# guiga-zalu/pixlzr-rust

Hardware: AMD Instinct MI355X
Metric: encode megapixels/sec (per-tile LOD detection + block-wise downsample), 8K RGBA (higher is better)
Workload: dtype u8

## Files before the change

### pixlzr-rust_amd/csrc/pxz_device.h

```cpp
#pragma once
#include <hip/hip_runtime.h>
#include <stdint.h>
#include <stdlib.h>

#include "pxz_internal.h"

namespace pxz {


static __constant__ uint32_t kSrgbToLinearBits[256] = {
#include "srgb_lut.inc"
};

struct RecipAlphaTable {
	uint32_t v[256];
	constexpr RecipAlphaTable() : v{}
	{
		for (uint32_t a = 1; a < 256; ++a) v[a] = ((255u * 512u) / a + 1u) >> 1;
	}
};
static __constant__ RecipAlphaTable kRecipAlpha = RecipAlphaTable();


__device__ __forceinline__ uint32_t fastdiv(uint32_t n, const FastDiv &d)
// ... 519 lines not shown
}

template <int C = 4>
__device__ __forceinline__ void resample_fast16_hv(const uint32_t *trows, const AxisTab &tx, const AxisTab &ty, const uint32_t *s_pl,
                                                   uint32_t *s_tmp, uint32_t lane, uint32_t nw, uint32_t nh, uint32_t *out)
{
	const uint32_t lgx = 31u - (uint32_t)__builtin_clz(nw);
	if (nw >= 4) {
		switch (tx.wquads) {
		case 1: fast32_h_pairs<1>(trows, tx, s_pl, s_tmp, lane, nw, lgx, 8u); break;
		case 2: fast32_h_pairs<2>(trows, tx, s_pl, s_tmp, lane, nw, lgx, 8u); break;
		case 3: fast32_h_pairs<3>(trows, tx, s_pl, s_tmp, lane, nw, lgx, 8u); break;
		default: fast32_h_pairs<4>(trows, tx, s_pl, s_tmp, lane, nw, lgx, 8u); break;
		}
	} else if (nw == 2) {
		fast32_h_rows<2>(trows, tx, s_pl, s_tmp, lane, nw, lgx, 16u);
	} else {
		fast32_h_rows<4>(trows, tx, s_pl, s_tmp, lane, nw, lgx, 16u);
	}
	tile_sync<1>();
	const uint32_t items = nw * nh;
	if (items >= 64u) fast32_v<1, C>(trows, tx, ty, s_tmp, lane, nw, nh, out);
	else if (items >= 32u) fast32_v<2, C>(trows, tx, ty, s_tmp, lane, nw, nh, out);
	else if (items >= 16u) fast32_v<4, C>(trows, tx, ty, s_tmp, lane, nw, nh, out);
	else fast32_v<8, C>(trows, tx, ty, s_tmp, lane, nw, nh, out);
	tile_sync<1>();
}

typedef int v4i32 __attribute__((ext_vector_type(4)));
typedef float f32x2 __attribute__((ext_vector_type(2)));

template <int BYTE>
__device__ __forceinline__ void put_byte_shr(uint32_t &dst, uint32_t value, uint32_t shift)
{
	if constexpr (BYTE == 0)
		asm("v_lshrrev_b32_sdwa %0, %1, %2 dst_sel:BYTE_0 dst_unused:UNUSED_PRESERVE src0_sel:DWORD src1_sel:DWORD" : "+v"(dst) : "v"(shift), "v"(value));
	else if constexpr (BYTE == 1)
		asm("v_lshrrev_b32_sdwa %0, %1, %2 dst_sel:BYTE_1 dst_unused:UNUSED_PRESERVE src0_sel:DWORD src1_sel:DWORD" : "+v"(dst) : "v"(shift), "v"(value));
	else if constexpr (BYTE == 2)
		asm("v_lshrrev_b32_sdwa %0, %1, %2 dst_sel:BYTE_2 dst_unused:UNUSED_PRESERVE src0_sel:DWORD src1_sel:DWORD" : "+v"(dst) : "v"(shift), "v"(value));
	else
		asm("v_lshrrev_b32_sdwa %0, %1, %2 dst_sel:BYTE_3 dst_unused:UNUSED_PRESERVE src0_sel:DWORD src1_sel:DWORD" : "+v"(dst) : "v"(shift), "v"(value));
}

__device__ __forceinline__ uint32_t clamp_fixed(int32_t hi, int32_t lo, int32_t top)
{
	const int32_t v = (int32_t)(((uint32_t)hi << 8) + (uint32_t)lo);
	int32_t r;
	asm("v_med3_i32 %0, %1, 0, %2" : "=v"(r) : "v"(v), "s"(top));
	return (uint32_t)r;
}

template <int NCH>
__device__ __forceinline__ void resample_mfma32(const uint32_t *s_tab, const AxisTab &tx, const AxisTab &ty, const uint32_t *s_pl,
                                                uint32_t lane, uint32_t nw, uint32_t nh, uint32_t *out)
{
	const uint32_t o = lane & 15u, g = lane >> 4;
	const uint32_t *mx = s_tab + tx.mf_off, *my = s_tab + ty.mf_off;
	const long kx_lo = *reinterpret_cast<const long *>(mx + 2u * lane), kx_hi = *reinterpret_cast<const long *>(mx + 128u + 2u * lane);
	const long ky_lo = *reinterpret_cast<const long *>(my + 2u * lane), ky_hi = *reinterpret_cast<const long *>(my + 128u + 2u * lane);
	const int32_t bx = (int32_t)mx[256u + o];
	const v4i32 cx = {bx, bx, bx, bx};
	const v4i32 cy = *reinterpret_cast<const v4i32 *>(my + 256u + 4u * g);
	const v4i32 zero = {0, 0, 0, 0};
	const uint32_t px_ = tx.precision, py = ty.precision;
	const int32_t top_x = (int32_t)((256u << px_) - 1u), top_y = (int32_t)((256u << py) - 1u);
	uint32_t pix[4] = {0xff000000u, 0xff000000u, 0xff000000u, 0xff000000u};
	const uint32_t *rowp = s_pl + o * kRS32 + 2u * g;
#pragma unroll
	for (uint32_t c = 0; c < (uint32_t)NCH; ++c) {
		uint32_t t[2];
#pragma unroll
		for (uint32_t mb = 0; mb < 2; ++mb) {
			const uint32_t *row = rowp + c * kPD32 + mb * (16u * kRS32);
			const uint2 d0 = lds_load2(row);
			const uint2 d1 = lds_load2(row + 8u);
			const uint32_t a0 = __builtin_amdgcn_perm(d0.y, d0.x, 0x06040200u) ^ 0x80808080u;
			const uint32_t a1 = __builtin_amdgcn_perm(d1.y, d1.x, 0x06040200u) ^ 0x80808080u;
			const long av = (long)(((unsigned long long)a1 << 32) | (unsigned long long)a0);
			const v4i32 lo = __builtin_amdgcn_mfma_i32_16x16x32_i8(av, kx_lo, cx, 0, 0, 0);
			const v4i32 hi = __builtin_amdgcn_mfma_i32_16x16x32_i8(av, kx_hi, zero, 0, 0, 0);
			uint32_t packed = 0;
			put_byte_shr<0>(packed, clamp_fixed(hi[0], lo[0], top_x), px_);
			put_byte_shr<1>(packed, clamp_fixed(hi[1], lo[1], top_x), px_);
			put_byte_shr<2>(packed, clamp_fixed(hi[2], lo[2], top_x), px_);
			put_byte_shr<3>(packed, clamp_fixed(hi[3], lo[3], top_x), px_);
			t[mb] = packed ^ 0x80808080u;
		}
		const long tv = (long)(((unsigned long long)t[1] << 32) | (unsigned long long)t[0]);
		const v4i32 lo = __builtin_amdgcn_mfma_i32_16x16x32_i8(ky_lo, tv, cy, 0, 0, 0);
		const v4i32 hi = __builtin_amdgcn_mfma_i32_16x16x32_i8(ky_hi, tv, zero, 0, 0, 0);
#pragma unroll
		for (int r = 0; r < 4; ++r) {
			const uint32_t v = clamp_fixed(hi[r], lo[r], top_y);
			if (c == 0) put_byte_shr<0>(pix[r], v, py);
			else if (c == 1) put_byte_shr<1>(pix[r], v, py);
			else if (c == 2) put_byte_shr<2>(pix[r], v, py);
			else put_byte_shr<3>(pix[r], v, py);
		}
	}
	if constexpr (NCH == 4) {
#pragma unroll
		for (int r = 0; r < 4; ++r) pix[r] = unpremultiply(pix[r]);
	} else if (!(mx[288] & my[288])) {
		const int32_t ah = (int32_t)clip8((1 << (px_ - 1)) + 255 * (int32_t)mx[272u + o], (int)px_);
#pragma unroll
		for (int r = 0; r < 4; ++r) {
			const uint32_t al = clip8((1 << (py - 1)) + ah * (int32_t)my[272u + 4u * g + (uint32_t)r], (int)py);
			pix[r] = (pix[r] & 0x00ffffffu) | (al << 24);
			if (al != 255u) pix[r] = unpremultiply(pix[r]);
		}
	}
	if (o < nw) {
#pragma unroll
		for (uint32_t r = 0; r < 4; ++r) {
			const uint32_t oy = 4u * g + r;
			if (oy < nh) out[oy * nw + o] = pix[r];
		}
	}
}

__device__ __forceinline__ void resample_mfma32_narrow(const uint32_t *s_tab, const AxisTab &tx, const AxisTab &ty, const uint32_t *s_pl,
                                                       uint32_t lane, uint32_t nw, uint32_t nh, uint32_t *out)
{
	const uint32_t o = lane & 15u, g = lane >> 4;
	const uint32_t lgw = nw >> 1;
	const uint32_t ch = o >> lgw, ox = o & (nw - 1u);
	const uint32_t *mx = s_tab + tx.mf_off, *my = s_tab + ty.mf_off;
	const uint32_t own = 2u * (16u * g + ox), none = 2u * (16u * g + 15u);
	const long ky_lo = *reinterpret_cast<const long *>(my + 2u * lane), ky_hi = *reinterpret_cast<const long *>(my + 128u + 2u * lane);
	const uint32_t px_ = tx.precision, py = ty.precision;
	const int32_t top_x = (int32_t)((256u << px_) - 1u), top_y = (int32_t)((256u << py) - 1u);
	const int32_t bx = ch == 3u ? top_x : (int32_t)mx[256u + ox];
	const v4i32 cy = *reinterpret_cast<const v4i32 *>(my + 256u + 4u * g);
	const v4i32 zero = {0, 0, 0, 0};
	v4i32 lo[2] = {{bx, bx, bx, bx}, {bx, bx, bx, bx}}, hi[2] = {zero, zero};
	const uint32_t *rowp = s_pl + o * kRS32 + 2u * g;
#pragma unroll
	for (uint32_t c = 0; c < 3; ++c) {
		const uint32_t sel = ch == c ? own : none;
		const long k_lo = *reinterpret_cast<const long *>(mx + sel), k_hi = *reinterpret_cast<const long *>(mx + 128u + sel);
#pragma unroll
		for (uint32_t mb = 0; mb < 2; ++mb) {
			const uint32_t *row = rowp + c * kPD32 + mb * (16u * kRS32);
			const uint2 d0 = lds_load2(row);
			const uint2 d1 = lds_load2(row + 8u);
			const uint32_t a0 = __builtin_amdgcn_perm(d0.y, d0.x, 0x06040200u) ^ 0x80808080u;
			const uint32_t a1 = __builtin_amdgcn_perm(d1.y, d1.x, 0x06040200u) ^ 0x80808080u;
			const long av = (long)(((unsigned long long)a1 << 32) | (unsigned long long)a0);
			lo[mb] = __builtin_amdgcn_mfma_i32_16x16x32_i8(av, k_lo, lo[mb], 0, 0, 0);
			hi[mb] = __builtin_amdgcn_mfma_i32_16x16x32_i8(av, k_hi, hi[mb], 0, 0, 0);
		}
	}
	uint32_t t[2];
#pragma unroll
	for (uint32_t mb = 0; mb < 2; ++mb) {
		uint32_t packed = 0;
		put_byte_shr<0>(packed, clamp_fixed(hi[mb][0], lo[mb][0], top_x), px_);
		put_byte_shr<1>(packed, clamp_fixed(hi[mb][1], lo[mb][1], top_x), px_);
		put_byte_shr<2>(packed, clamp_fixed(hi[mb][2], lo[mb][2], top_x), px_);
		put_byte_shr<3>(packed, clamp_fixed(hi[mb][3], lo[mb][3], top_x), px_);
		t[mb] = packed ^ 0x80808080u;
	}
	const long tv = (long)(((unsigned long long)t[1] << 32) | (unsigned long long)t[0]);
	const v4i32 vlo = __builtin_amdgcn_mfma_i32_16x16x32_i8(ky_lo, tv, cy, 0, 0, 0);
	const v4i32 vhi = __builtin_amdgcn_mfma_i32_16x16x32_i8(ky_hi, tv, zero, 0, 0, 0);
	if (o < 4u * nw && 4u * g < nh) {
		uint8_t *dst = reinterpret_cast<uint8_t *>(out) + (4u * g * nw + ox) * 4u + ch;
		dst[0] = (uint8_t)(clamp_fixed(vhi[0], vlo[0], top_y) >> py);
		if (nh > 1u) dst[nw * 4u] = (uint8_t)(clamp_fixed(vhi[1], vlo[1], top_y) >> py);
		if (nh > 2u) {
			dst[2u * nw * 4u] = (uint8_t)(clamp_fixed(vhi[2], vlo[2], top_y) >> py);
			dst[3u * nw * 4u] = (uint8_t)(clamp_fixed(vhi[3], vlo[3], top_y) >> py);
		}
	}
}

__device__ __forceinline__ uint32_t clamp_fixed_v(int32_t hi, int32_t lo, int32_t top)
{
	const int32_t v = (int32_t)(((uint32_t)hi << 8) + (uint32_t)lo);
	int32_t r;
	asm("v_med3_i32 %0, %1, 0, %2" : "=v"(r) : "v"(v), "v"(top));
	return (uint32_t)r;
}
// ... 46 lines not shown
			const v4i32 cx = {bx[mb], bx[mb], bx[mb], bx[mb]};
			const v4i32 lo = __builtin_amdgcn_mfma_i32_16x16x32_i8(av, kx_lo[mb], cx, 0, 0, 0);
			const v4i32 hi = __builtin_amdgcn_mfma_i32_16x16x32_i8(av, kx_hi[mb], zero, 0, 0, 0);
			uint32_t packed = 0;
			put_byte_shr<0>(packed, clamp_fixed_v(hi[0], lo[0], top_x[mb]), px_[mb]);
			put_byte_shr<1>(packed, clamp_fixed_v(hi[1], lo[1], top_x[mb]), px_[mb]);
			put_byte_shr<2>(packed, clamp_fixed_v(hi[2], lo[2], top_x[mb]), px_[mb]);
			put_byte_shr<3>(packed, clamp_fixed_v(hi[3], lo[3], top_x[mb]), px_[mb]);
			t[mb] = packed ^ 0x80808080u;
		}
		const uint32_t l0 = second ? 0u : t[0], l1 = second ? 0u : t[1], r0 = second ? t[0] : 0u, r1 = second ? t[1] : 0u;
		const long tl = (long)(((unsigned long long)l1 << 32) | (unsigned long long)l0);
		const long tr = (long)(((unsigned long long)r1 << 32) | (unsigned long long)r0);
		v4i32 lo = __builtin_amdgcn_mfma_i32_16x16x32_i8(ky_lo[0], tl, cy, 0, 0, 0);
		lo = __builtin_amdgcn_mfma_i32_16x16x32_i8(ky_lo[1], tr, lo, 0, 0, 0);
		v4i32 hi = __builtin_amdgcn_mfma_i32_16x16x32_i8(ky_hi[0], tl, zero, 0, 0, 0);
		hi = __builtin_amdgcn_mfma_i32_16x16x32_i8(ky_hi[1], tr, hi, 0, 0, 0);
#pragma unroll
		for (int r = 0; r < 4; ++r) {
			const uint32_t v = clamp_fixed_v(hi[r], lo[r], top_y);
			if (c == 0) put_byte_shr<0>(pix[r], v, py);
			else if (c == 1) put_byte_shr<1>(pix[r], v, py);
			else put_byte_shr<2>(pix[r], v, py);
		}
	}
	if (ok && o < nw) {
#pragma unroll
		for (uint32_t r = 0; r < 4; ++r) {
			const uint32_t oy = 4u * (g & 1u) + r;
			if (oy < nh) store_pixel<C>(dst, oy * nw + o, pix[r]);
		}
	}
}

__device__ __forceinline__ uint4 stream_load4(const uint8_t *p)
{
	typedef uint32_t u32q __attribute__((ext_vector_type(4)));
	const u32q v = __builtin_nontemporal_load(reinterpret_cast<const u32q *>(p));
	return make_uint4(v.x, v.y, v.z, v.w);
}
__device__ __forceinline__ uint2 stream_load2(const uint8_t *p)
{
	typedef uint32_t u32d __attribute__((ext_vector_type(2)));
	const u32d v = __builtin_nontemporal_load(reinterpret_cast<const u32d *>(p));
	return make_uint2(v.x, v.y);
}
__device__ __forceinline__ uint3 stream_load3(const uint8_t *p)
{
	typedef uint32_t u32t __attribute__((ext_vector_type(3)));
	const u32t v = __builtin_nontemporal_load(reinterpret_cast<const u32t *>(p));
	return make_uint3(v.x, v.y, v.z);
}

template <int C = 4, class Args>
__device__ __forceinline__ bool fast32_tile_src(const Args &a, uint32_t tile_g, const uint8_t *&src)
{
	if (tile_g >= a.n_tiles) return false;
	const uint32_t frame = fastdiv(tile_g, a.div_tpf);
	const uint32_t t = tile_g - frame * a.tiles_per_frame;
	const uint32_t ty = fastdiv(t, a.div_cols), tx = t - ty * a.cols;
	src = a.src + (size_t)frame * a.frame_stride + (size_t)(ty * 32u) * a.pitch + (size_t)(tx * 32u) * (uint32_t)C;
	return tx < a.full_cols && ty < a.full_rows;
}
template <int C = 4, class Args>
__device__ __forceinline__ void fast32_prefetch(const Args &a, uint32_t tile_g, uint32_t lane, uint4 (&pre)[4], bool &valid, bool skip_loads = false)
{
	const uint8_t *src;
	valid = fast32_tile_src<C>(a, tile_g, src);
	if (valid && !skip_loads) {
		const uint8_t *p = src + (size_t)(lane >> 3) * a.pitch + (lane & 7u) * (4u * (uint32_t)C);
#pragma unroll
		for (int k = 0; k < 4; ++k) {
			if constexpr (C == 4) {
				pre[k] = stream_load4(p + (size_t)(8 * k) * a.pitch);
			} else {
				const uint3 v = stream_load3(p + (size_t)(8 * k) * a.pitch);
				pre[k] = make_uint4(v.x, v.y, v.z, 0u);
			}
		}
	}
}

template <class Args>
__device__ __forceinline__ bool oklab_value_given(const Args &a, uint32_t tx, uint32_t ty)
{
	const bool in_x = tx < a.full_cols, in_y = ty < a.full_rows;
	if (in_x && ty < a.ok_rows) return true;
	const uint32_t bit = in_x ? 2u : (in_y ? 1u : 4u);
	return (a.ok_edges & bit) != 0u;
}

constexpr uint32_t kDeferredKey = 0xffffffffu;
__device__ __forceinline__ void finish_tile(const uint2 key, uint32_t w, uint32_t h, uint32_t mode, float factor, float *value,
                                            float *lod0, float *lod1, uint32_t tile_g)
{
	float raw0, raw1, v0, v1;
	if (mode == 1) {
		const uint64_t fac = (uint64_t)(w - 2) * (uint64_t)(h - 2) * 4096ull;
		if (fac == 0) {
			raw0 = raw1 = __uint_as_float(0xFFC00000u);
			v0 = v1 = 0.0f;
		} else {
			const double d = (double)fac;
			raw0 = (float)((double)key.x / d);
			raw1 = (float)((double)key.y / d);
			v0 = parse_value(raw0 * factor);
			v1 = parse_value(raw1 * factor);
		}
	} else {
		raw0 = raw1 = __uint_as_float(key.x);
		v0 = v1 = parse_value(raw0);
	}
	if (value) value[tile_g] = hypot_f32(v0, v1);
	if (lod0) lod0[tile_g] = raw0;
	if (lod1) lod1[tile_g] = raw1;
}

#ifdef PXZ_STAMPS
__device__ __forceinline__ unsigned long long stamp_now()
{
	unsigned long long t;
	__builtin_amdgcn_sched_barrier(0);
	asm volatile("s_memtime %0\n\ts_waitcnt lgkmcnt(0)" : "=s"(t)::"memory");
	__builtin_amdgcn_sched_barrier(0);
	return t;
}
#define PXZ_STAMP(i)                                   \
	do {                                               \
		const unsigned long long now_ = stamp_now();   \
		st_acc[i] += now_ - st_last;                   \
		st_last = now_;                                \
	} while (0)
#else
// ... 241 lines not shown
```

### pixlzr-rust_amd/csrc/pxz_shrink32.hip

```cpp
#include "pxz_device.h"

namespace pxz {


template <int MODE, bool FULL, int C = 4>
__global__ void __launch_bounds__(1024) shrink32_kernel(const Fast32Args a)
{
	extern __shared__ __attribute__((aligned(16))) uint32_t lds[];
	const uint32_t wpb = blockDim.x / 64u, sub = threadIdx.x / 64u, tid = threadIdx.x % 64u;
	for (uint32_t i = threadIdx.x; i < a.tab_dw / 4u; i += blockDim.x)
		reinterpret_cast<uint4 *>(lds)[i] = reinterpret_cast<const uint4 *>(a.trows)[i];
	uint32_t *s_ticket = lds + a.tab_dw + wpb * a.tile_dw;
	if (threadIdx.x == 0) *s_ticket = wpb;
	__syncthreads();
	const uint32_t *s_tab = lds;
	const uint32_t brk_lane = tid < (uint32_t)kMaxLevel ? a.breaks[tid] : (a.breaks_asc ? 0xffffffffu : 0u);
	auto level_of = [&](uint32_t key) -> uint32_t {
		const unsigned long long lt = __builtin_amdgcn_ballot_w64(key < brk_lane);
		const unsigned long long live = (1ull << kMaxLevel) - 1ull;
		return (uint32_t)__builtin_popcountll((a.breaks_asc ? ~lt : lt) & live);
	};
	uint32_t *s_pl = lds + a.tab_dw + sub * a.tile_dw;
	uint32_t *s_tmp = s_pl + 3 * kPD32;
	uint32_t *s_batch = s_ticket + 4u + sub * (2u * kListBatch);
	uint32_t n_listb = 0, n_lista = 0;
	auto tile_of_ticket = [&](uint32_t t) -> uint32_t {
		const unsigned long long run = (unsigned long long)(t >> a.chunk_lg) * gridDim.x + blockIdx.x;
		const unsigned long long g = (run << a.chunk_lg) + (t & ((1u << a.chunk_lg) - 1u));
		return g < (unsigned long long)a.n_tiles ? (uint32_t)g : 0xffffffffu;
	};
	auto next_ticket = [&]() -> uint32_t {
		uint32_t t = 0;
		if (tid == 0) t = atomicAdd(s_ticket, 1u);
		return tile_of_ticket(__builtin_amdgcn_readfirstlane(t));
	};
	uint4 pre[4];
	bool pre_valid = false;
	const uint32_t first = tile_of_ticket(__builtin_amdgcn_readfirstlane(sub));
	bool pre_skipped = false;
	uint32_t vb_cur = 0, vb_next = 0;
	uint32_t fl_next = 0;
	auto value_pair_of = [&](uint32_t t) -> uint2 { return t < a.n_tiles ? reinterpret_cast<const uint2 *>(a.sums)[t] : make_uint2(0u, 0u); };
	auto stored_whole = [&](uint32_t vb, uint32_t copied) -> bool {
		return a.clone_ahead && copied == 1u && level_of(__float_as_uint(parse_value(__uint_as_float(vb)))) == 0u;
	};
	uint32_t second = 0xffffffffu;
	if constexpr (MODE == 0) {
		second = next_ticket();
		const uint2 p0 = value_pair_of(first), p1 = value_pair_of(second);
		vb_cur = __builtin_amdgcn_readfirstlane(p0.x);
		vb_next = __builtin_amdgcn_readfirstlane(p1.x);
		fl_next = __builtin_amdgcn_readfirstlane(p1.y);
		pre_skipped = stored_whole(vb_cur, __builtin_amdgcn_readfirstlane(p0.y));
		fast32_prefetch<C>(a, first, tid, pre, pre_valid, pre_skipped);
	} else {
		fast32_prefetch<C>(a, first, tid, pre, pre_valid);
	}
#ifdef PXZ_STAMPS
	unsigned long long st_acc[8] = {0, 0, 0, 0, 0, 0, 0, 0};
	unsigned long long st_last = stamp_now();
	const unsigned long long st_begin = wall_clock64();
#endif
	uint32_t pend_kind = 0;
	uint32_t pend_px = 0;
	const uint32_t *pend_src = nullptr;
	uint8_t *pend_dst = nullptr;
	auto flush = [&]() {
		if (pend_kind == 1) {
			if constexpr (C == 4) {
				uint32_t *d = reinterpret_cast<uint32_t *>(pend_dst);
				if (pend_px >= 4u) {
					for (uint32_t i = tid; i < (pend_px >> 2); i += 64u)
						reinterpret_cast<uint4 *>(d)[i] = reinterpret_cast<const uint4 *>(pend_src)[i];
				} else if (tid < pend_px) {
					d[tid] = pend_src[tid];
				}
			} else {
				if (pend_px >= 4u) {
					for (uint32_t i = tid; i < (pend_px >> 2); i += 64u) {
						const uint4 v = reinterpret_cast<const uint4 *>(pend_src)[i];
						uint3 o;
						o.x = __builtin_amdgcn_perm(v.y, v.x, 0x04020100u);
						o.y = __builtin_amdgcn_perm(v.z, v.y, 0x05040201u);
						o.z = __builtin_amdgcn_perm(v.w, v.z, 0x06050402u);
						reinterpret_cast<uint3 *>(pend_dst)[i] = o;
					}
				} else if (tid < pend_px) {
					const uint32_t v = pend_src[tid];
					pend_dst[3u * tid] = (uint8_t)v;
					pend_dst[3u * tid + 1u] = (uint8_t)(v >> 8);
					pend_dst[3u * tid + 2u] = (uint8_t)(v >> 16);
				}
			}
		} else if (pend_kind == 2) {
#pragma unroll
			for (int k = 0; k < 4; ++k) {
				const uint32_t i = tid + 64u * (uint32_t)k;
				const uint32_t *p = s_pl + (i >> 3) * kRS32 + (i & 7u) * 2u;
				const uint2 r = *reinterpret_cast<const uint2 *>(p), g = *reinterpret_cast<const uint2 *>(p + kPD32);
				const uint2 b = *reinterpret_cast<const uint2 *>(p + 2 * kPD32);
				const uint32_t rg01 = __builtin_amdgcn_perm(g.x, r.x, 0x06020400u), rg23 = __builtin_amdgcn_perm(g.y, r.y, 0x06020400u);
				if constexpr (C == 4) {
					const uint32_t opq = 0x00ff00ffu;
					const uint32_t ba01 = __builtin_amdgcn_perm(opq, b.x, 0x06020400u), ba23 = __builtin_amdgcn_perm(opq, b.y, 0x06020400u);
					uint4 o;
					o.x = __builtin_amdgcn_perm(ba01, rg01, 0x05040100u);
					o.y = __builtin_amdgcn_perm(ba01, rg01, 0x07060302u);
					o.z = __builtin_amdgcn_perm(ba23, rg23, 0x05040100u);
					o.w = __builtin_amdgcn_perm(ba23, rg23, 0x07060302u);
					reinterpret_cast<uint4 *>(pend_dst)[i] = o;
				} else {
					uint3 o;
					o.x = __builtin_amdgcn_perm(b.x, rg01, 0x02040100u);
					const uint32_t gb1 = __builtin_amdgcn_perm(b.x, rg01, 0x0c0c0603u);
					o.y = __builtin_amdgcn_perm(rg23, gb1, 0x05040100u);
					o.z = __builtin_amdgcn_perm(b.y, rg23, 0x06030204u);
					reinterpret_cast<uint3 *>(pend_dst)[i] = o;
				}
			}
		}
		pend_kind = 0;
	};
	auto one_tile = [&](const uint32_t tile_g, const uint32_t tile_next) {
		auto prefetch_next = [&]() __attribute__((always_inline)) {
			if constexpr (MODE == 0) {
				pre_skipped = stored_whole(vb_next, fl_next);
				fast32_prefetch<C>(a, tile_next, tid, pre, pre_valid, pre_skipped);
			} else {
				fast32_prefetch<C>(a, tile_next, tid, pre, pre_valid);
			}
		};
		auto defer = [&]() {
			list_push(s_batch, n_listb, tile_g, a.work + kWorkList, a.work + a.work_slot, tid);
			if (tid == 0) {
				bool keep = false;
				if constexpr (MODE == 0) {
					const uint32_t t = tile_g - fastdiv(tile_g, a.div_tpf) * a.tiles_per_frame;
					const uint32_t ty = fastdiv(t, a.div_cols), tx = t - ty * a.cols;
					keep = oklab_value_given(a, tx, ty);
				}
				if (!keep) reinterpret_cast<uint2 *>(a.sums)[tile_g] = make_uint2(kDeferredKey, kDeferredKey);
			}
		};
		if (!pre_valid) {
			flush();
			defer();
			prefetch_next();
			return;
		}
		uint32_t given_bits = 0;
		if constexpr (MODE == 0) given_bits = vb_cur;
		const bool skipped = MODE == 0 && pre_skipped;
		bool transparent = false;
		if (C == 4 && !skipped) {
			uint32_t least;
			const uint32_t m0 = min(min(pre[0].x, pre[0].y), pre[0].z), m1 = min(min(pre[0].w, pre[1].x), pre[1].y);
			const uint32_t m2 = min(min(pre[1].z, pre[1].w), pre[2].x), m3 = min(min(pre[2].y, pre[2].z), pre[2].w);
			const uint32_t m4 = min(min(pre[3].x, pre[3].y), pre[3].z);
			least = min(min(min(m0, m1), m2), min(min(m3, m4), pre[3].w));
			transparent = __builtin_amdgcn_ballot_w64(least < 0xff000000u) != 0ull;
		}
		__builtin_amdgcn_sched_barrier(0);
		flush();
		__builtin_amdgcn_sched_barrier(0);
		if (!skipped) {
#pragma unroll
		for (int k = 0; k < 4; ++k) {
			const uint32_t row = (tid >> 3) + 8u * (uint32_t)k, col = tid & 7u;
			const uint4 v = pre[k];
			uint32_t *d = s_pl + row * kRS32 + col * 2u;
			if constexpr (C == 4) {
#pragma unroll
				for (uint32_t c = 0; c < 3; ++c) {
					const uint32_t sel = c | 0x0c000c00u | ((4u + c) << 16);
					uint2 pr;
					pr.x = __builtin_amdgcn_perm(v.y, v.x, sel);
					pr.y = __builtin_amdgcn_perm(v.w, v.z, sel);
					lds_store2(d + c * kPD32, pr);
				}
			} else {
				lds_store2(d, make_uint2(__builtin_amdgcn_perm(v.x, v.x, 0x0c070c00u), __builtin_amdgcn_perm(v.z, v.y, 0x0c050c02u)));
				lds_store2(d + kPD32, make_uint2(__builtin_amdgcn_perm(v.y, v.x, 0x0c040c01u), __builtin_amdgcn_perm(v.z, v.y, 0x0c060c03u)));
				lds_store2(d + 2 * kPD32, make_uint2(__builtin_amdgcn_perm(v.y, v.x, 0x0c050c02u), __builtin_amdgcn_perm(v.z, v.z, 0x0c070c00u)));
			}
		}
		}
		PXZ_STAMP(0);
		prefetch_next();
		if (skipped) {
			uint32_t lane = tid;
			asm volatile("" : "+v"(lane));
			if (lane == 0) {
				if (FULL || a.out_w) a.out_w[tile_g] = 32u;
				if (FULL || a.out_h) a.out_h[tile_g] = 32u;
			}
			return;
		}
		if (transparent && (FULL || a.out_px != nullptr)) {
			if (a.alpha_list) {
				list_push(s_batch + kListBatch, n_lista, tile_g, a.work + kWorkList + a.n_tiles, a.work + kWorkA + a.work_slot, tid);
				if constexpr (MODE == 1)
					if (tid == 0) reinterpret_cast<uint2 *>(a.sums)[tile_g] = make_uint2(kDeferredKey, kDeferredKey);
			} else {
				defer();
			}
			return;
		}
		tile_sync<1>();
		PXZ_STAMP(1);

		uint32_t m0, m1;
		uint32_t key0 = 0, key1 = 0;
		if constexpr (MODE == 1) {
			uint32_t sum_hz = 0, sum_vr = 0;
			const uint32_t q = tid & 15u, g = tid >> 4;
			auto last_rows = [](uint32_t grp) -> bool {
				asm volatile("" : "+v"(grp));
				return grp != 3u;
			};
			const uint32_t two = 0x00020002u;
			const uint32_t *pc[3];
			pc[0] = s_pl + g * (8u * kRS32) + q;
			pc[1] = pc[0] + kPD32;
			pc[2] = pc[1] + kPD32;
			uint32_t rA[3], rB[3], tP[3], dP[3];
#pragma unroll
			for (int c = 0; c < 3; ++c) {
				const uint32_t a0 = lds_dword(pc[0] + c * kPD32), a1 = lds_dword(pc[0] + c * kPD32 + 1);
				const uint32_t b0 = lds_dword(pc[0] + c * kPD32 + kRS32), b1 = lds_dword(pc[0] + c * kPD32 + kRS32 + 1);
				rA[c] = pk_mad_u16(__builtin_amdgcn_alignbit(a1, a0, 16), two, add2x16(a0, a1));
				rB[c] = pk_mad_u16(__builtin_amdgcn_alignbit(b1, b0, 16), two, add2x16(b0, b1));
				tP[c] = add2x16(a0, b0);
				dP[c] = b0;
			}
#pragma unroll
			for (int st = 0; st < 4; ++st) {
				if (st < 3 || last_rows(g)) {
#pragma unroll
					for (int c = 0; c < 3; ++c) {
						const uint32_t *pr = pc[0] + c * kPD32 + (2 + 2 * st) * (int)kRS32;
						const uint32_t n0 = lds_dword(pr), n1 = lds_dword(pr + 1), o0 = lds_dword(pr + kRS32), o1 = lds_dword(pr + kRS32 + 1);
						const uint32_t rN = pk_mad_u16(__builtin_amdgcn_alignbit(n1, n0, 16), two, add2x16(n0, n1));
						sum_hz = sad16(rN, rA[c], sum_hz);
						const uint32_t tN = add2x16(dP[c], n0);
						const uint32_t c0 = add2x16(tP[c], tN);
						sum_vr = sad16(dpp_mov<0x101>(c0), c0, sum_vr);
						const uint32_t rO = pk_mad_u16(__builtin_amdgcn_alignbit(o1, o0, 16), two, add2x16(o0, o1));
						sum_hz = sad16(rO, rB[c], sum_hz);
						const uint32_t tO = add2x16(n0, o0);
						const uint32_t e0 = add2x16(tN, tO);
						sum_vr = sad16(dpp_mov<0x101>(e0), e0, sum_vr);
						rA[c] = rN;
						rB[c] = rO;
						tP[c] = tO;
						dP[c] = o0;
					}
				}
			}
			{
				uint32_t qq = q;
				asm volatile("" : "+v"(qq));
				if (qq == 15u) sum_hz = sum_vr = 0;
			}
			sum_hz = wave_sum_sgpr(sum_hz);
			sum_vr = wave_sum_sgpr(sum_vr);
			m0 = level_of(sum_hz);
			m1 = level_of(sum_vr);
			key0 = sum_hz;
			key1 = sum_vr;
		} else {
			m0 = m1 = level_of(__float_as_uint(parse_value(__uint_as_float(given_bits))));
		}
		const uint32_t nw = reduced_size(32u, m0), nh = reduced_size(32u, m1);
		{
			uint32_t lane = tid;
			asm volatile("" : "+v"(lane));
			if (lane == 0) {
				if constexpr (MODE == 1) reinterpret_cast<uint2 *>(a.sums)[tile_g] = make_uint2(key0, key1);
				if (FULL || a.out_w) a.out_w[tile_g] = nw;
				if (FULL || a.out_h) a.out_h[tile_g] = nh;
			}
		}
		PXZ_STAMP(2);
		if (FULL || a.out_px != nullptr) {
			uint32_t filt = a.filter;
			asm volatile("" : "+s"(filt));
			pend_dst = a.out_px + (size_t)tile_g * (1024u * (uint32_t)C);
			pend_px = nw * nh;
			if (nw == 32u && nh == 32u) {
				pend_kind = 2;
			} else if (nw != 32u && nh != 32u && filt != 0) {
				const uint32_t lx = m0 < (uint32_t)kMaxLevel ? m0 : (uint32_t)kMaxLevel - 1;
				const uint32_t ly = m1 < (uint32_t)kMaxLevel ? m1 : (uint32_t)kMaxLevel - 1;
				const bool both_mf = a.tabs[lx].mf_off != 0 && a.tabs[ly].mf_off != 0;
				if (a.narrow && both_mf && nw <= 4u && nh <= 16u && (s_tab[a.tabs[lx].mf_off + 288u] & s_tab[a.tabs[ly].mf_off + 288u])) {
					resample_mfma32_narrow(s_tab, a.tabs[lx], a.tabs[ly], s_pl, tid, nw, nh, s_tmp);
					pend_src = s_tmp;
					pend_kind = 1;
				} else if (both_mf && nw >= 4u && nh >= 4u) {
					resample_mfma32<3>(s_tab, a.tabs[lx], a.tabs[ly], s_pl, tid, nw, nh, s_tmp);
					pend_src = s_tmp;
					pend_kind = 1;
				} else if (nw <= 8u) {
					resample_fast32_hv(s_tab, a.tabs[lx], a.tabs[ly], s_pl, s_tmp, tid, nw, nh, s_pl);
					pend_src = s_pl;
					pend_kind = 1;
				} else {
					defer();
				}
			} else if (filt == 0) {
				const uint32_t lgx = 31u - (uint32_t)__builtin_clz(nw);
				const uint32_t hx = m0 ? (1u << (m0 < 6u ? m0 - 1u : 4u)) : 0u, hy = m1 ? (1u << (m1 < 6u ? m1 - 1u : 4u)) : 0u;
				const uint16_t *pl16 = reinterpret_cast<const uint16_t *>(s_pl);
				for (uint32_t i = tid; i < nw * nh; i += 64u) {
					const uint32_t ox = i & (nw - 1u), oy = i >> lgx;
					const uint32_t x = m0 == 0 ? ox : (m0 < 6u ? (2u * ox + 1u) * hx : 16u);
					const uint32_t y = m1 == 0 ? oy : (m1 < 6u ? (2u * oy + 1u) * hy : 16u);
					const uint32_t idx = y * (2u * kRS32) + x;
					s_tmp[i] = (uint32_t)pl16[idx] | ((uint32_t)pl16[idx + 2u * kPD32] << 8) | ((uint32_t)pl16[idx + 4u * kPD32] << 16) | 0xff000000u;
				}
				pend_kind = 1;
				pend_src = s_tmp;
			} else if (nh != 32u) {
				const uint32_t ly = m1 < (uint32_t)kMaxLevel ? m1 : (uint32_t)kMaxLevel - 1;
				fast32_v_only(s_tab, a.tabs[ly], s_pl, tid, nh, s_tmp);
				pend_kind = 1;
				pend_src = s_tmp;
			} else {
				const uint32_t lx = m0 < (uint32_t)kMaxLevel ? m0 : (uint32_t)kMaxLevel - 1;
				fast32_h_only(s_tab, a.tabs[lx], s_pl, tid, nw, s_tmp);
				pend_kind = 1;
				pend_src = s_tmp;
			}
		}
		tile_sync<1>();
		PXZ_STAMP(3);
	};
#ifdef PXZ_STAMPS
	uint32_t st_tiles = 0;
#endif
	for (uint32_t tile_g = first, tile_next = second; tile_g < a.n_tiles;) {
#ifdef PXZ_STAMPS
		++st_tiles;
#endif
		if constexpr (MODE == 0) {
			const uint32_t tile_after = next_ticket();
			const uint2 pair_after = value_pair_of(tile_after);
			one_tile(tile_g, tile_next);
			tile_g = tile_next;
			tile_next = tile_after;
			vb_cur = vb_next;
			vb_next = __builtin_amdgcn_readfirstlane(pair_after.x);
			fl_next = __builtin_amdgcn_readfirstlane(pair_after.y);
		} else {
			tile_next = next_ticket();
			one_tile(tile_g, tile_next);
			tile_g = tile_next;
		}
	}
#ifdef PXZ_STAMPS
	unsigned long long st_loop_end;
	asm volatile("s_memrealtime %0\n\ts_waitcnt lgkmcnt(0)" : "=s"(st_loop_end)::"memory");
#endif
	flush();
	list_flush(s_batch, n_listb, a.work + kWorkList, a.work + a.work_slot, tid);
	list_flush(s_batch + kListBatch, n_lista, a.work + kWorkList + a.n_tiles, a.work + kWorkA + a.work_slot, tid);
	if (a.finish_here) {
		__threadfence_block();
		__syncthreads();
		for (uint32_t i = threadIdx.x;; i += blockDim.x) {
			const unsigned long long run = (unsigned long long)(i >> a.chunk_lg) * gridDim.x + blockIdx.x;
			const unsigned long long g = (run << a.chunk_lg) + (i & ((1u << a.chunk_lg) - 1u));
			if (g >= (unsigned long long)a.n_tiles) break;
			const uint2 key = reinterpret_cast<const uint2 *>(a.sums)[g];
			if (key.x == kDeferredKey && key.y == kDeferredKey) continue;
			finish_tile(key, 32u, 32u, (uint32_t)MODE, a.factor, a.value, a.lod0, a.lod1, (uint32_t)g);
		}
	}
#ifdef PXZ_STAMPS
	if (tid == 0) {
		unsigned long long *out = reinterpret_cast<unsigned long long *>(a.work + ((2u * a.n_tiles + kWorkList + 1u + 1u) & ~1u));
		for (int i = 0; i < 8; ++i) atomicAdd(out + i, st_acc[i]);
// ... 20 lines not shown
		const unsigned long long live = (1ull << kMaxLevel) - 1ull;
		return (uint32_t)__builtin_popcountll((a.breaks_asc ? ~lt : lt) & live);
	};
	uint32_t *s_pl = lds + a.tab_dw + sub * a.tile_dw;
	uint32_t *s_batch = s_ticket + 4u + sub * kListBatch;
	uint32_t n_listb = 0;
	const uint32_t count = a.all_tiles ? a.n_tiles : __builtin_amdgcn_readfirstlane(a.work[kWorkA + a.work_slot]);
	const uint32_t *list = a.work + kWorkList + a.n_tiles;
	uint32_t n_transparent = 0;
	auto tile_of_ticket = [&](uint32_t t) -> uint32_t {
		const unsigned long long i = (unsigned long long)blockIdx.x + (unsigned long long)t * gridDim.x;
		return i < (unsigned long long)count ? (a.all_tiles ? (uint32_t)i : list[(uint32_t)i]) : 0xffffffffu;
	};
	auto next_ticket = [&]() -> uint32_t {
		uint32_t t = 0;
		if (tid == 0) t = atomicAdd(s_ticket, 1u);
		return __builtin_amdgcn_readfirstlane(tile_of_ticket(__builtin_amdgcn_readfirstlane(t)));
	};
	uint4 pre[4];
	bool pre_valid = false;
	const uint32_t first = __builtin_amdgcn_readfirstlane(tile_of_ticket(__builtin_amdgcn_readfirstlane(sub)));
	fast32_prefetch(a, first, tid, pre, pre_valid);
	for (uint32_t tile_g = first; tile_g < a.n_tiles;) {
		const uint32_t tile_next = next_ticket();
		auto defer = [&]() {
			list_push(s_batch, n_listb, tile_g, a.work + kWorkList, a.work + a.work_slot, tid);
		};
		if (!pre_valid) {
			if (tid == 0) {
				bool keep = false;
				if constexpr (MODE == 0) {
					const uint32_t t = tile_g - fastdiv(tile_g, a.div_tpf) * a.tiles_per_frame;
					const uint32_t ty = fastdiv(t, a.div_cols), tx = t - ty * a.cols;
					keep = oklab_value_given(a, tx, ty);
				}
				if (!keep) reinterpret_cast<uint2 *>(a.sums)[tile_g] = make_uint2(kDeferredKey, kDeferredKey);
			}
			defer();
			fast32_prefetch(a, tile_next, tid, pre, pre_valid);
			tile_g = tile_next;
			continue;
		}
		uint32_t given_bits = 0;
		if constexpr (MODE == 0) given_bits = a.sums[2 * tile_g];
		if (a.all_tiles) {
			const uint32_t m0 = min(min(pre[0].x, pre[0].y), pre[0].z), m1 = min(min(pre[0].w, pre[1].x), pre[1].y);
			const uint32_t m2 = min(min(pre[1].z, pre[1].w), pre[2].x), m3 = min(min(pre[2].y, pre[2].z), pre[2].w);
			const uint32_t m4 = min(min(pre[3].x, pre[3].y), pre[3].z);
			const uint32_t least = min(min(min(m0, m1), m2), min(min(m3, m4), pre[3].w));
			n_transparent += __builtin_amdgcn_ballot_w64(least < 0xff000000u) != 0ull ? 1u : 0u;
		}
#pragma unroll
		for (int k = 0; k < 4; ++k) {
			const uint32_t row = (tid >> 3) + 8u * (uint32_t)k, col = tid & 7u;
			const uint4 v = pre[k];
			uint32_t *d = s_pl + row * kRS32 + col * 2u;
#pragma unroll
			for (uint32_t c = 0; c < 4; ++c) {
				const uint32_t sel = c | 0x0c000c00u | ((4u + c) << 16);
				uint2 pr;
				pr.x = __builtin_amdgcn_perm(v.y, v.x, sel);
				pr.y = __builtin_amdgcn_perm(v.w, v.z, sel);
				lds_store2(d + c * kPD32, pr);
			}
		}
		fast32_prefetch(a, tile_next, tid, pre, pre_valid);
		tile_sync<1>();
		uint32_t m0, m1;
		if constexpr (MODE == 1) {
			uint32_t sum_hz = 0, sum_vr = 0;
			const uint32_t q = tid & 15u, g = tid >> 4;
			const uint32_t two = 0x00020002u;
			const uint32_t *pc[3];
			pc[0] = s_pl + g * (8u * kRS32) + q;
			pc[1] = pc[0] + kPD32;
			pc[2] = pc[1] + kPD32;
			uint32_t rA[3], rB[3], tP[3], dP[3];
#pragma unroll
			for (int c = 0; c < 3; ++c) {
				const uint32_t a0 = pc[c][0], a1 = pc[c][1], b0 = pc[c][kRS32], b1 = pc[c][kRS32 + 1];
				rA[c] = pk_mad_u16(__builtin_amdgcn_alignbit(a1, a0, 16), two, add2x16(a0, a1));
				rB[c] = pk_mad_u16(__builtin_amdgcn_alignbit(b1, b0, 16), two, add2x16(b0, b1));
				tP[c] = add2x16(a0, b0);
				dP[c] = b0;
			}
#pragma unroll
			for (int st = 0; st < 4; ++st) {
				if (st < 3 || g != 3u) {
#pragma unroll
					for (int c = 0; c < 3; ++c) {
						const uint32_t *pr = pc[c] + (2 + 2 * st) * (int)kRS32;
						const uint32_t n0 = pr[0], n1 = pr[1], o0 = pr[kRS32], o1 = pr[kRS32 + 1];
						const uint32_t rN = pk_mad_u16(__builtin_amdgcn_alignbit(n1, n0, 16), two, add2x16(n0, n1));
						sum_hz = sad16(rN, rA[c], sum_hz);
						const uint32_t tN = add2x16(dP[c], n0);
						const uint32_t c0 = add2x16(tP[c], tN);
						sum_vr = sad16(dpp_mov<0x101>(c0), c0, sum_vr);
						const uint32_t rO = pk_mad_u16(__builtin_amdgcn_alignbit(o1, o0, 16), two, add2x16(o0, o1));
						sum_hz = sad16(rO, rB[c], sum_hz);
						const uint32_t tO = add2x16(n0, o0);
						const uint32_t e0 = add2x16(tN, tO);
						sum_vr = sad16(dpp_mov<0x101>(e0), e0, sum_vr);
						rA[c] = rN;
						rB[c] = rO;
						tP[c] = tO;
						dP[c] = o0;
					}
// ... 18 lines not shown
			tile_sync<1>();
			tile_g = tile_next;
			continue;
		}
		if (tid == 0) {
			if (a.out_w) a.out_w[tile_g] = nw;
			if (a.out_h) a.out_h[tile_g] = nh;
		}
		uint32_t *dst = reinterpret_cast<uint32_t *>(a.out_px + (size_t)tile_g * 4096u);
		if (nw == 32u && nh == 32u) {
#pragma unroll
			for (int k = 0; k < 4; ++k) {
				const uint32_t i = tid + 64u * (uint32_t)k;
				const uint32_t *p = s_pl + (i >> 3) * kRS32 + (i & 7u) * 2u;
				const uint2 r = *reinterpret_cast<const uint2 *>(p), g = *reinterpret_cast<const uint2 *>(p + kPD32);
				const uint2 b = *reinterpret_cast<const uint2 *>(p + 2 * kPD32), al = *reinterpret_cast<const uint2 *>(p + 3 * kPD32);
				const uint32_t rg01 = __builtin_amdgcn_perm(g.x, r.x, 0x06020400u), ba01 = __builtin_amdgcn_perm(al.x, b.x, 0x06020400u);
				const uint32_t rg23 = __builtin_amdgcn_perm(g.y, r.y, 0x06020400u), ba23 = __builtin_amdgcn_perm(al.y, b.y, 0x06020400u);
				uint4 o;
				o.x = __builtin_amdgcn_perm(ba01, rg01, 0x05040100u);
				o.y = __builtin_amdgcn_perm(ba01, rg01, 0x07060302u);
				o.z = __builtin_amdgcn_perm(ba23, rg23, 0x05040100u);
				o.w = __builtin_amdgcn_perm(ba23, rg23, 0x07060302u);
				reinterpret_cast<uint4 *>(dst)[i] = o;
			}
		} else if (a.filter == 0) {
			const uint32_t lgx = 31u - (uint32_t)__builtin_clz(nw);
			const uint32_t hx = m0 ? (1u << (m0 < 6u ? m0 - 1u : 4u)) : 0u, hy = m1 ? (1u << (m1 < 6u ? m1 - 1u : 4u)) : 0u;
			const uint16_t *pl16 = reinterpret_cast<const uint16_t *>(s_pl);
			for (uint32_t i = tid; i < nw * nh; i += 64u) {
				const uint32_t ox = i & (nw - 1u), oy = i >> lgx;
				const uint32_t x = m0 == 0 ? ox : (m0 < 6u ? (2u * ox + 1u) * hx : 16u);
				const uint32_t y = m1 == 0 ? oy : (m1 < 6u ? (2u * oy + 1u) * hy : 16u);
				const uint32_t idx = y * (2u * kRS32) + x;
				dst[i] = (uint32_t)pl16[idx] | ((uint32_t)pl16[idx + 2u * kPD32] << 8) | ((uint32_t)pl16[idx + 4u * kPD32] << 16) |
				         ((uint32_t)pl16[idx + 6u * kPD32] << 24);
			}
		} else {
#pragma unroll
			for (uint32_t it = 0; it < 8; ++it) {
				const uint32_t i = tid + 64u * it;
				uint32_t *p = s_pl + (i >> 4) * kRS32 + (i & 15u);
				const ushort2v al = us2(p[3 * kPD32]);
#pragma unroll
				for (uint32_t c = 0; c < 3; ++c) {
					ushort2v t = us2(p[c * kPD32]) * al + (ushort2v)(128);
					t = t + (t >> (ushort2v)(8));
					p[c * kPD32] = u32(t >> (ushort2v)(8));
				}
			}
			tile_sync<1>();
			const uint32_t lx = m0 < (uint32_t)kMaxLevel ? m0 : (uint32_t)kMaxLevel - 1;
			const uint32_t ly = m1 < (uint32_t)kMaxLevel ? m1 : (uint32_t)kMaxLevel - 1;
			resample_mfma32<4>(s_tab, a.tabs[lx], a.tabs[ly], s_pl, tid, nw, nh, dst);
		}
		tile_sync<1>();
		tile_g = tile_next;
	}
	list_flush(s_batch, n_listb, a.work + kWorkList, a.work + a.work_slot, tid);
	if (a.all_tiles && n_transparent != 0u && tid == 0) atomicAdd(a.work + kWorkA + a.work_slot, n_transparent);
}

template <int MODE, bool FULL, int C = 4>
__global__ void __launch_bounds__(1024) shrink16_kernel(const Fast32Args a)
{
	extern __shared__ __attribute__((aligned(16))) uint32_t lds[];
	const uint32_t wpb = blockDim.x / 64u, sub = threadIdx.x / 64u, tid = threadIdx.x % 64u;
	for (uint32_t i = threadIdx.x; i < a.tab_dw / 4u; i += blockDim.x)
		reinterpret_cast<uint4 *>(lds)[i] = reinterpret_cast<const uint4 *>(a.trows)[i];
	uint32_t *s_ticket = lds + a.tab_dw + wpb * a.tile_dw;
	if (threadIdx.x == 0) *s_ticket = wpb;
	__syncthreads();
	const uint32_t *s_tab = lds;
	const uint32_t brk_lane = tid < (uint32_t)kMaxLevel ? a.breaks[tid] : (a.breaks_asc ? 0xffffffffu : 0u);
	auto level_of = [&](uint32_t key) -> uint32_t {
		const unsigned long long lt = __builtin_amdgcn_ballot_w64(key < brk_lane);
		const unsigned long long live = (1ull << kMaxLevel) - 1ull;
		return (uint32_t)__builtin_popcountll((a.breaks_asc ? ~lt : lt) & live);
	};
	uint32_t *s_pl = lds + a.tab_dw + sub * a.tile_dw;
	uint32_t *s_tmp = s_pl + 3 * kPD32;
	uint32_t *s_batch = s_ticket + 4u + sub * kListBatch;
	uint32_t n_listb = 0;
	const uint32_t gcols = (a.cols + 1u) >> 1, grows = (a.rows + 1u) >> 1, gpf = gcols * grows;
	auto group_of_ticket = [&](uint32_t t) -> uint32_t {
		const unsigned long long run = (unsigned long long)(t >> a.chunk_lg) * gridDim.x + blockIdx.x;
		const unsigned long long g = (run << a.chunk_lg) + (t & ((1u << a.chunk_lg) - 1u));
		return g < (unsigned long long)a.n_groups ? (uint32_t)g : 0xffffffffu;
	};
	auto next_ticket = [&]() -> uint32_t {
		uint32_t t = 0;
		if (tid == 0) t = atomicAdd(s_ticket, 1u);
		return group_of_ticket(__builtin_amdgcn_readfirstlane(t));
	};
	struct Place {
		uint32_t frame, gx, gy;
		bool full;
		const uint8_t *src;
	};
	auto place_of = [&](uint32_t grp) -> Place {
		Place p{0, 0, 0, false, nullptr};
		if (grp >= a.n_groups) return p;
		p.frame = fastdiv(grp, a.div_gpf);
		const uint32_t r = grp - p.frame * gpf;
		p.gy = fastdiv(r, a.div_gcols);
		p.gx = r - p.gy * gcols;
		p.src = a.src + (size_t)p.frame * a.frame_stride + (size_t)(p.gy * 32u) * a.pitch + (size_t)(p.gx * 32u) * (uint32_t)C;
// ... 456 lines not shown
```

Before: 1.106 million.

## Pack per-level tables into lane registers and reorder tile-load row mapping

Per-level resample parameters (table offset, precision, alpha-stays flag, filter/narrow/alpha-list flags) and tile geometry are packed into one register per lane at kernel start and fetched with readlane. This replaces repeated scalar and LDS loads of kernel arguments and tables in the per-tile loop. The global-load row mapping per lane is also permuted so each wavefront load instruction touches a different row pattern, which may change coalescing and cache behaviour. It adds register pressure and readlane latency, and the row remap must stay consistent between the load and LDS-store sides.

```diff
diff --git a/pixlzr-rust_amd/csrc/pxz_device.h b/pixlzr-rust_amd/csrc/pxz_device.h
--- a/pixlzr-rust_amd/csrc/pxz_device.h
+++ b/pixlzr-rust_amd/csrc/pxz_device.h
@@ -595,18 +595,17 @@
 }
 
 template <int NCH>
-__device__ __forceinline__ void resample_mfma32(const uint32_t *s_tab, const AxisTab &tx, const AxisTab &ty, const uint32_t *s_pl,
-                                                uint32_t lane, uint32_t nw, uint32_t nh, uint32_t *out)
+__device__ __forceinline__ void resample_mfma32(const uint32_t *s_tab, uint32_t mf_x, uint32_t mf_y, uint32_t px_, uint32_t py, bool alpha_stays,
+                                                const uint32_t *s_pl, uint32_t lane, uint32_t nw, uint32_t nh, uint32_t *out)
 {
 	const uint32_t o = lane & 15u, g = lane >> 4;
-	const uint32_t *mx = s_tab + tx.mf_off, *my = s_tab + ty.mf_off;
+	const uint32_t *mx = s_tab + mf_x, *my = s_tab + mf_y;
 	const long kx_lo = *reinterpret_cast<const long *>(mx + 2u * lane), kx_hi = *reinterpret_cast<const long *>(mx + 128u + 2u * lane);
 	const long ky_lo = *reinterpret_cast<const long *>(my + 2u * lane), ky_hi = *reinterpret_cast<const long *>(my + 128u + 2u * lane);
 	const int32_t bx = (int32_t)mx[256u + o];
 	const v4i32 cx = {bx, bx, bx, bx};
 	const v4i32 cy = *reinterpret_cast<const v4i32 *>(my + 256u + 4u * g);
 	const v4i32 zero = {0, 0, 0, 0};
-	const uint32_t px_ = tx.precision, py = ty.precision;
 	const int32_t top_x = (int32_t)((256u << px_) - 1u), top_y = (int32_t)((256u << py) - 1u);
 	uint32_t pix[4] = {0xff000000u, 0xff000000u, 0xff000000u, 0xff000000u};
 	const uint32_t *rowp = s_pl + o * kRS32 + 2u * g;
@@ -645,7 +644,7 @@
 	if constexpr (NCH == 4) {
 #pragma unroll
 		for (int r = 0; r < 4; ++r) pix[r] = unpremultiply(pix[r]);
-	} else if (!(mx[288] & my[288])) {
+	} else if (!alpha_stays) {
 		const int32_t ah = (int32_t)clip8((1 << (px_ - 1)) + 255 * (int32_t)mx[272u + o], (int)px_);
 #pragma unroll
 		for (int r = 0; r < 4; ++r) {
@@ -663,16 +662,15 @@
 	}
 }
 
-__device__ __forceinline__ void resample_mfma32_narrow(const uint32_t *s_tab, const AxisTab &tx, const AxisTab &ty, const uint32_t *s_pl,
-                                                       uint32_t lane, uint32_t nw, uint32_t nh, uint32_t *out)
+__device__ __forceinline__ void resample_mfma32_narrow(const uint32_t *s_tab, uint32_t mf_x, uint32_t mf_y, uint32_t px_, uint32_t py,
+                                                       const uint32_t *s_pl, uint32_t lane, uint32_t nw, uint32_t nh, uint32_t *out)
 {
 	const uint32_t o = lane & 15u, g = lane >> 4;
 	const uint32_t lgw = nw >> 1;
 	const uint32_t ch = o >> lgw, ox = o & (nw - 1u);
-	const uint32_t *mx = s_tab + tx.mf_off, *my = s_tab + ty.mf_off;
+	const uint32_t *mx = s_tab + mf_x, *my = s_tab + mf_y;
 	const uint32_t own = 2u * (16u * g + ox), none = 2u * (16u * g + 15u);
 	const long ky_lo = *reinterpret_cast<const long *>(my + 2u * lane), ky_hi = *reinterpret_cast<const long *>(my + 128u + 2u * lane);
-	const uint32_t px_ = tx.precision, py = ty.precision;
 	const int32_t top_x = (int32_t)((256u << px_) - 1u), top_y = (int32_t)((256u << py) - 1u);
 	const int32_t bx = ch == 3u ? top_x : (int32_t)mx[256u + ox];
 	const v4i32 cy = *reinterpret_cast<const v4i32 *>(my + 256u + 4u * g);
@@ -825,33 +823,73 @@
 	return make_uint3(v.x, v.y, v.z);
 }
 
+struct Fast32Geom {
+	uint32_t cols, pitch, full_cols, full_rows;
+};
 template <int C = 4, class Args>
-__device__ __forceinline__ bool fast32_tile_src(const Args &a, uint32_t tile_g, const uint8_t *&src)
+__device__ __forceinline__ bool fast32_tile_src(const Args &a, uint32_t tile_g, const uint8_t *&src, const Fast32Geom &gm)
 {
 	if (tile_g >= a.n_tiles) return false;
 	const uint32_t frame = fastdiv(tile_g, a.div_tpf);
 	const uint32_t t = tile_g - frame * a.tiles_per_frame;
-	const uint32_t ty = fastdiv(t, a.div_cols), tx = t - ty * a.cols;
-	src = a.src + (size_t)frame * a.frame_stride + (size_t)(ty * 32u) * a.pitch + (size_t)(tx * 32u) * (uint32_t)C;
-	return tx < a.full_cols && ty < a.full_rows;
+	const uint32_t ty = fastdiv(t, a.div_cols), tx = t - ty * gm.cols;
+	src = a.src + (size_t)frame * a.frame_stride + (size_t)(ty * 32u) * gm.pitch + (size_t)(tx * 32u) * (uint32_t)C;
+	return tx < gm.full_cols && ty < gm.full_rows;
+}
+template <int C = 4, class Args>
+__device__ __forceinline__ bool fast32_tile_src(const Args &a, uint32_t tile_g, const uint8_t *&src)
+{
+	return fast32_tile_src<C>(a, tile_g, src, Fast32Geom{a.cols, a.pitch, a.full_cols, a.full_rows});
+}
+__device__ __forceinline__ uint32_t fast32_lane_row(uint32_t lane, uint32_t k)
+{
+	return ((lane >> 3) & 1u) * 8u + (lane >> 4) + 4u * (k & 1u) + 16u * (k >> 1);
+}
+template <int C = 4, class Args>
+__device__ __forceinline__ void fast32_prefetch(const Args &a, uint32_t tile_g, uint32_t lane, uint4 (&pre)[4], bool &valid, bool skip_loads,
+                                                const Fast32Geom &gm)
+{
+	const uint8_t *src;
+	valid = fast32_tile_src<C>(a, tile_g, src, gm);
+	if (valid && !skip_loads) {
+		const uint8_t *p = src + (size_t)fast32_lane_row(lane, 0u) * gm.pitch + (lane & 7u) * (4u * (uint32_t)C);
+#pragma unroll
+		for (uint32_t k = 0; k < 4; ++k) {
+			const size_t down = (size_t)fast32_lane_row(0u, k) * gm.pitch;
+			if constexpr (C == 4) {
+				pre[k] = stream_load4(p + down);
+			} else {
+				const uint3 v = stream_load3(p + down);
+				pre[k] = make_uint4(v.x, v.y, v.z, 0u);
+			}
+		}
+	}
 }
 template <int C = 4, class Args>
 __device__ __forceinline__ void fast32_prefetch(const Args &a, uint32_t tile_g, uint32_t lane, uint4 (&pre)[4], bool &valid, bool skip_loads = false)
 {
-	const uint8_t *src;
-	valid = fast32_tile_src<C>(a, tile_g, src);
-	if (valid && !skip_loads) {
-		const uint8_t *p = src + (size_t)(lane >> 3) * a.pitch + (lane & 7u) * (4u * (uint32_t)C);
-#pragma unroll
-		for (int k = 0; k < 4; ++k) {
-			if constexpr (C == 4) {
-				pre[k] = stream_load4(p + (size_t)(8 * k) * a.pitch);
-			} else {
-				const uint3 v = stream_load3(p + (size_t)(8 * k) * a.pitch);
-				pre[k] = make_uint4(v.x, v.y, v.z, 0u);
-			}
-		}
-	}
+	fast32_prefetch<C>(a, tile_g, lane, pre, valid, skip_loads, Fast32Geom{a.cols, a.pitch, a.full_cols, a.full_rows});
+}
+
+constexpr uint32_t kLvMfMask = 0xffffu, kLvPrecShift = 16u, kLvPrecMask = 0x1fu;
+constexpr uint32_t kLvStays = 1u << 21;
+constexpr uint32_t kLvFilter = 1u << 24;
+constexpr uint32_t kLvNarrow = 1u << 25;
+constexpr uint32_t kLvAlphaList = 1u << 26;
+constexpr uint32_t kLvCols = (uint32_t)kMaxLevel, kLvPitch = kLvCols + 1u, kLvFullCols = kLvCols + 2u, kLvFullRows = kLvCols + 3u;
+template <class Args>
+__device__ __forceinline__ uint32_t level_pack(const Args &a, const uint32_t *s_tab, uint32_t lane)
+{
+	uint32_t v = 0;
+	if (lane < (uint32_t)kMaxLevel) {
+		const uint32_t mf = a.tabs[lane].mf_off;
+		v = (mf & kLvMfMask) | (((uint32_t)a.tabs[lane].precision & kLvPrecMask) << kLvPrecShift);
+		if (mf != 0u && s_tab[mf + 288u] != 0u) v |= kLvStays;
+		v |= (a.filter != 0u ? kLvFilter : 0u) | (a.narrow != 0u ? kLvNarrow : 0u) | (a.alpha_list != 0u ? kLvAlphaList : 0u);
+	} else if (lane <= kLvFullRows) {
+		v = lane == kLvCols ? a.cols : (lane == kLvPitch ? a.pitch : (lane == kLvFullCols ? a.full_cols : a.full_rows));
+	}
+	return v;
 }
 
 template <class Args>
diff --git a/pixlzr-rust_amd/csrc/pxz_shrink32.hip b/pixlzr-rust_amd/csrc/pxz_shrink32.hip
--- a/pixlzr-rust_amd/csrc/pxz_shrink32.hip
+++ b/pixlzr-rust_amd/csrc/pxz_shrink32.hip
@@ -20,6 +20,9 @@
 		const unsigned long long live = (1ull << kMaxLevel) - 1ull;
 		return (uint32_t)__builtin_popcountll((a.breaks_asc ? ~lt : lt) & live);
 	};
+	const uint32_t lvl_lane = level_pack(a, s_tab, tid);
+	auto lvl_of = [&](uint32_t l) -> uint32_t { return (uint32_t)__builtin_amdgcn_readlane((int)lvl_lane, (int)l); };
+	auto geom = [&]() -> Fast32Geom { return Fast32Geom{lvl_of(kLvCols), lvl_of(kLvPitch), lvl_of(kLvFullCols), lvl_of(kLvFullRows)}; };
 	uint32_t *s_pl = lds + a.tab_dw + sub * a.tile_dw;
 	uint32_t *s_tmp = s_pl + 3 * kPD32;
 	uint32_t *s_batch = s_ticket + 4u + sub * (2u * kListBatch);
@@ -52,9 +55,9 @@
 		vb_next = __builtin_amdgcn_readfirstlane(p1.x);
 		fl_next = __builtin_amdgcn_readfirstlane(p1.y);
 		pre_skipped = stored_whole(vb_cur, __builtin_amdgcn_readfirstlane(p0.y));
-		fast32_prefetch<C>(a, first, tid, pre, pre_valid, pre_skipped);
+		fast32_prefetch<C>(a, first, tid, pre, pre_valid, pre_skipped, geom());
 	} else {
-		fast32_prefetch<C>(a, first, tid, pre, pre_valid);
+		fast32_prefetch<C>(a, first, tid, pre, pre_valid, false, geom());
 	}
 #ifdef PXZ_STAMPS
 	unsigned long long st_acc[8] = {0, 0, 0, 0, 0, 0, 0, 0};
@@ -125,9 +128,9 @@
 		auto prefetch_next = [&]() __attribute__((always_inline)) {
 			if constexpr (MODE == 0) {
 				pre_skipped = stored_whole(vb_next, fl_next);
-				fast32_prefetch<C>(a, tile_next, tid, pre, pre_valid, pre_skipped);
+				fast32_prefetch<C>(a, tile_next, tid, pre, pre_valid, pre_skipped, geom());
 			} else {
-				fast32_prefetch<C>(a, tile_next, tid, pre, pre_valid);
+				fast32_prefetch<C>(a, tile_next, tid, pre, pre_valid, false, geom());
 			}
 		};
 		auto defer = [&]() {
@@ -166,7 +169,7 @@
 		if (!skipped) {
 #pragma unroll
 		for (int k = 0; k < 4; ++k) {
-			const uint32_t row = (tid >> 3) + 8u * (uint32_t)k, col = tid & 7u;
+			const uint32_t row = fast32_lane_row(tid, (uint32_t)k), col = tid & 7u;
 			const uint4 v = pre[k];
 			uint32_t *d = s_pl + row * kRS32 + col * 2u;
 			if constexpr (C == 4) {
@@ -197,7 +200,7 @@
 			return;
 		}
 		if (transparent && (FULL || a.out_px != nullptr)) {
-			if (a.alpha_list) {
+			if (lvl_of(0u) & kLvAlphaList) {
 				list_push(s_batch + kListBatch, n_lista, tile_g, a.work + kWorkList + a.n_tiles, a.work + kWorkA + a.work_slot, tid);
 				if constexpr (MODE == 1)
 					if (tid == 0) reinterpret_cast<uint2 *>(a.sums)[tile_g] = make_uint2(kDeferredKey, kDeferredKey);
@@ -283,22 +286,25 @@
 		}
 		PXZ_STAMP(2);
 		if (FULL || a.out_px != nullptr) {
-			uint32_t filt = a.filter;
-			asm volatile("" : "+s"(filt));
+			const uint32_t lx = m0 < (uint32_t)kMaxLevel ? m0 : (uint32_t)kMaxLevel - 1;
+			const uint32_t ly = m1 < (uint32_t)kMaxLevel ? m1 : (uint32_t)kMaxLevel - 1;
+			const uint32_t sx = lvl_of(lx), sy = lvl_of(ly);
+			const bool filt = (sx & kLvFilter) != 0u;
 			pend_dst = a.out_px + (size_t)tile_g * (1024u * (uint32_t)C);
 			pend_px = nw * nh;
 			if (nw == 32u && nh == 32u) {
 				pend_kind = 2;
-			} else if (nw != 32u && nh != 32u && filt != 0) {
-				const uint32_t lx = m0 < (uint32_t)kMaxLevel ? m0 : (uint32_t)kMaxLevel - 1;
-				const uint32_t ly = m1 < (uint32_t)kMaxLevel ? m1 : (uint32_t)kMaxLevel - 1;
-				const bool both_mf = a.tabs[lx].mf_off != 0 && a.tabs[ly].mf_off != 0;
-				if (a.narrow && both_mf && nw <= 4u && nh <= 16u && (s_tab[a.tabs[lx].mf_off + 288u] & s_tab[a.tabs[ly].mf_off + 288u])) {
-					resample_mfma32_narrow(s_tab, a.tabs[lx], a.tabs[ly], s_pl, tid, nw, nh, s_tmp);
+			} else if (nw != 32u && nh != 32u && filt) {
+				const uint32_t mf_x = sx & kLvMfMask, mf_y = sy & kLvMfMask;
+				const uint32_t prec_x = (sx >> kLvPrecShift) & kLvPrecMask, prec_y = (sy >> kLvPrecShift) & kLvPrecMask;
+				const bool both_mf = mf_x != 0u && mf_y != 0u;
+				const bool stays = (sx & sy & kLvStays) != 0u;
+				if ((sx & kLvNarrow) && both_mf && nw <= 4u && nh <= 16u && stays) {
+					resample_mfma32_narrow(s_tab, mf_x, mf_y, prec_x, prec_y, s_pl, tid, nw, nh, s_tmp);
 					pend_src = s_tmp;
 					pend_kind = 1;
 				} else if (both_mf && nw >= 4u && nh >= 4u) {
-					resample_mfma32<3>(s_tab, a.tabs[lx], a.tabs[ly], s_pl, tid, nw, nh, s_tmp);
+					resample_mfma32<3>(s_tab, mf_x, mf_y, prec_x, prec_y, stays, s_pl, tid, nw, nh, s_tmp);
 					pend_src = s_tmp;
 					pend_kind = 1;
 				} else if (nw <= 8u) {
@@ -308,7 +314,7 @@
 				} else {
 					defer();
 				}
-			} else if (filt == 0) {
+			} else if (!filt) {
 				const uint32_t lgx = 31u - (uint32_t)__builtin_clz(nw);
 				const uint32_t hx = m0 ? (1u << (m0 < 6u ? m0 - 1u : 4u)) : 0u, hy = m1 ? (1u << (m1 < 6u ? m1 - 1u : 4u)) : 0u;
 				const uint16_t *pl16 = reinterpret_cast<const uint16_t *>(s_pl);
@@ -322,12 +328,10 @@
 				pend_kind = 1;
 				pend_src = s_tmp;
 			} else if (nh != 32u) {
-				const uint32_t ly = m1 < (uint32_t)kMaxLevel ? m1 : (uint32_t)kMaxLevel - 1;
 				fast32_v_only(s_tab, a.tabs[ly], s_pl, tid, nh, s_tmp);
 				pend_kind = 1;
 				pend_src = s_tmp;
 			} else {
-				const uint32_t lx = m0 < (uint32_t)kMaxLevel ? m0 : (uint32_t)kMaxLevel - 1;
 				fast32_h_only(s_tab, a.tabs[lx], s_pl, tid, nw, s_tmp);
 				pend_kind = 1;
 				pend_src = s_tmp;
@@ -454,7 +458,7 @@
 		}
 #pragma unroll
 		for (int k = 0; k < 4; ++k) {
-			const uint32_t row = (tid >> 3) + 8u * (uint32_t)k, col = tid & 7u;
+			const uint32_t row = fast32_lane_row(tid, (uint32_t)k), col = tid & 7u;
 			const uint4 v = pre[k];
 			uint32_t *d = s_pl + row * kRS32 + col * 2u;
 #pragma unroll
@@ -579,7 +583,7 @@
 			tile_sync<1>();
 			const uint32_t lx = m0 < (uint32_t)kMaxLevel ? m0 : (uint32_t)kMaxLevel - 1;
 			const uint32_t ly = m1 < (uint32_t)kMaxLevel ? m1 : (uint32_t)kMaxLevel - 1;
-			resample_mfma32<4>(s_tab, a.tabs[lx], a.tabs[ly], s_pl, tid, nw, nh, dst);
+			resample_mfma32<4>(s_tab, a.tabs[lx].mf_off, a.tabs[ly].mf_off, a.tabs[lx].precision, a.tabs[ly].precision, false, s_pl, tid, nw, nh, dst);
 		}
 		tile_sync<1>();
 		tile_g = tile_next;
```

New measurement: 1.114 million (median of 6 runs). Within noise of the previous version (+0.7%).
